# Srujan-D/spectral

Hardware: AMD Instinct MI355X
Metric: trajectory QP solves/sec (20-seg order-5 corridor) (higher is better)
Workload: dtype f64

## Files before the change

spectral_amd/csrc/btrapz_device.h:

```cpp
#ifndef BTRAPZ_DEVICE_H
#define BTRAPZ_DEVICE_H

#include "../../include/btrapz_hip.h"

#define BTRAPZ_EXPORT extern "C" __attribute__((visibility("default")))

#define BTRAPZ_FAR 1e9
#define BTRAPZ_FAR_FACTOR 1048576.0
#define BTRAPZ_FAR_LIMIT 1e6
#define BTRAPZ_COLD_FAR 1e4

namespace btrapz {

struct Shared {
  double w_s[4], w_l[4];
  double weight_end_s, weight_end_l;
  double ds_ref, dl_ref;
  double acc_s[2];
  double acc_l[2];
  double jerk_s[2], jerk_l[2];
  int variant;
};

struct KernelArgs {
// ... 124 lines not shown
  double rate;
  double s_lo, s_hi, l_lo, l_hi, l_safe, w_safe;
};

struct CorridorArgs {
  int B, N, num_obs, variant, seg_stride;
  double delta;
  const double *s_bounds, *l_bounds;
  const double *prisms;
  int P;
  PrismRoad road;
  int *n_strips;
  const double *ds_bounds, *dl_bounds;
  const double *s_ref, *l_ref;
  double *seg;
  int *seg_count;
  double *ref_end;
  double *dl10;
  int cap_o, cap_sel;
  int pass;
  int *retry_list, *retry_count;
};

__global__ void corridor_batch_kernel(const CorridorArgs a, int staged);
__global__ void corridor_batch_short_kernel(const CorridorArgs a, int staged);
__global__ void corridor_first_kernel(const CorridorArgs a, int staged);
__global__ void corridor_first_short_kernel(const CorridorArgs a, int staged);
__global__ void prism_corridor_batch_kernel(const CorridorArgs a, int staged);
__global__ void prism_corridor_batch_short_kernel(const CorridorArgs a, int staged);
__global__ void prism_corridor_first_kernel(const CorridorArgs a, int staged);
__global__ void prism_corridor_first_short_kernel(const CorridorArgs a, int staged);
struct Seg;
__global__ void corridor_serial_kernel(const CorridorArgs a, Seg *ws_all, Seg *ws_sel);
struct CorridorVjpArgs {
  int B, N, num_obs, variant, seg_stride;
  double delta;
  const double *s_bounds, *l_bounds, *ds_bounds, *s_ref, *l_ref;
  const double *seg_bar, *ref_end_bar, *dl10_bar;
  btrapz_knot_grads out;
  int cap_o, cap_sel, pass, staged;
  int *retry_list, *retry_count;
};
constexpr int kCorridorVjpTerms = 16;
struct CorridorVjpLds { int rows; size_t sel, dyn, ints, bytes; };
__host__ __device__ inline CorridorVjpLds corridor_vjp_lds(int N, int O, int cap_o, int cap_sel, int seg_stride, int staged) {
  CorridorVjpLds l;
  const size_t cap_all = (size_t)cap_o * O, seg_bytes = 104;
  l.rows = (cap_sel < seg_stride ? cap_sel : seg_stride) + 1;
  const size_t terms = (size_t)kCorridorVjpTerms * l.rows * (sizeof(double) + sizeof(int));
  l.sel = ((seg_bytes * cap_all > terms ? seg_bytes * cap_all : terms) + 15) & ~(size_t)15;
  l.dyn = (l.sel + seg_bytes * cap_sel + 15) & ~(size_t)15;
  const size_t table = staged ? (size_t)O * N * 2 : 0, refs = (size_t)N * 4;
  l.ints = l.dyn + sizeof(double) * (table > refs ? table : refs);
  l.bytes = l.ints + sizeof(int) * (64 + 4) + sizeof(short) * (cap_all + cap_sel);
  return l;
}
__global__ void corridor_vjp_kernel(const CorridorVjpArgs a);
__global__ void prestart_kernel(const KernelArgs a, int S_uniform, const int *seg_count, int *keys);
__global__ void bucket_hist_kernel(int B, int seg_stride, const int *seg_count, int *meta, int fixed_S);
__global__ void bucket_prefix_kernel(int *meta, int fixed_S);
__global__ void bucket_scatter_kernel(int B, int seg_stride, const int *seg_count, int *meta, int *order,
                                      double *axis_obj, int *axis_status, int *axis_iters, int fixed_S);
__global__ void ipm_solve_kernel(const KernelArgs a, const double *__restrict__ mqm);
__global__ void ipm_solve_ordered_kernel(const KernelArgs a, const double *__restrict__ mqm);
__global__ void ipm_solve_warm_kernel(const KernelArgs a, const double *__restrict__ mqm);
__global__ void ipm_solve_warm_ordered_kernel(const KernelArgs a, const double *__restrict__ mqm);
#ifdef BTRAPZ_EXPERIMENTS
__global__ void ipm_solve_queue_kernel(const KernelArgs a, const double *__restrict__ mqm);
#endif
__global__ void ipm_solve_elastic_kernel(const KernelArgs a, const double *__restrict__ mqm);
__global__ void ipm_solve_split_kernel(const KernelArgs a, const double *__restrict__ mqm);
__global__ void ipm_solve_capped_kernel(const KernelArgs a, const double *__restrict__ mqm);
__global__ void ipm_solve_capped_ordered_kernel(const KernelArgs a, const double *__restrict__ mqm);
__global__ void ipm_solve_resume_kernel(const KernelArgs a, const double *__restrict__ mqm);
__global__ void ipm_solve_lean_kernel(const KernelArgs a, const double *__restrict__ mqm);
__global__ void ipm_solve_lean_ordered_kernel(const KernelArgs a, const double *__restrict__ mqm);
__global__ void ipm_solve_lean_capped_kernel(const KernelArgs a, const double *__restrict__ mqm);
__global__ void ipm_solve_lean_capped_ordered_kernel(const KernelArgs a, const double *__restrict__ mqm);
__global__ void ipm_solve_lean_resume_kernel(const KernelArgs a, const double *__restrict__ mqm);
__global__ void ipm_solve_lean_pipe_capped_kernel(const KernelArgs a, const double *__restrict__ mqm, int axis);
__global__ void ipm_solve_lean_pipe_resume_kernel(const KernelArgs a, const double *__restrict__ mqm, int axis);
__global__ void ipm_solve_lean_pipe_kernel(const KernelArgs a, const double *__restrict__ mqm, int n_resume, int resume_axis, int capped_axis);
__global__ void pipe_counts_kernel(const int *tables, volatile int *host_counts);
__global__ void ipm_solve_lean_warm_kernel(const KernelArgs a, const double *__restrict__ mqm);
__global__ void ipm_solve_lean_warm_ordered_kernel(const KernelArgs a, const double *__restrict__ mqm);
__global__ void ipm_solve_sets_ordered_kernel(const KernelArgs a, const double *__restrict__ mqm, const Shared *sets, int n_keys);
__global__ void ipm_solve_sets_warm_ordered_kernel(const KernelArgs a, const double *__restrict__ mqm, const Shared *sets, int n_keys);
__global__ void ipm_solve_lean_sets_ordered_kernel(const KernelArgs a, const double *__restrict__ mqm, const Shared *sets, int n_keys);
__global__ void ipm_solve_lean_sets_warm_ordered_kernel(const KernelArgs a, const double *__restrict__ mqm, const Shared *sets, int n_keys);
__global__ void ipm_solve_sets_split_kernel(const KernelArgs a, const double *__restrict__ mqm, const Shared *sets, const int *set_index, int n_sets);
__global__ void ipm_solve_long_sets_kernel(const KernelArgs a, const double *__restrict__ mqm, const Shared *sets, const int *set_index, int n_sets);
__global__ void sets_hist_kernel(int B, int seg_stride, const int *seg_count, const int *set_index, int n_sets, int n_keys, int *meta);
__global__ void sets_prefix_kernel(int n_keys, int fixed_S, int *meta);
__global__ void sets_scatter_kernel(int B, int seg_stride, const int *seg_count, const int *set_index, int n_sets, int n_keys,
                                    int *meta, int *order, double *axis_obj, int *axis_status, int *axis_iters);
#define BTRAPZ_SUSPENDED (-7)
__global__ void ipm_solve_long_kernel(const KernelArgs a, const double *__restrict__ mqm);
__global__ void ipm_solve_long_elastic_kernel(const KernelArgs a, const double *__restrict__ mqm);
__global__ void rescue_keys_kernel(int B, int S, const int *seg_count, const int *axis_status, int *keys, int all);
__global__ void rescue_init_kernel(int B, int S, const int *seg_count, double *axis_obj, int *axis_status, int *axis_iters);
struct MqmWeights { double w[2][4]; };
__global__ void mqm_table_kernel(MqmWeights w, double *out);
__global__ void mqm_sets_kernel(const Shared *sets, double *out);
__global__ void rescue_violations_kernel(int B, const double *axis_viol, double *viol);
__global__ void finalize_kernel(int B, const double *axis_obj, const int *axis_status, const int *axis_iters,
                                double *cost, int *status, int *iters);
__global__ void argmin_kernel(int group, long long index_base, const double *cost, long long *best_idx,
                              double *best_cost, double *part_cost, long long *part_idx);
__global__ void argmin_final_kernel(int chunks, long long index_base, const double *part_cost, const long long *part_idx,
                                    long long *best_idx, double *best_cost);
__global__ void argmin_pairs_kernel(int world, int n, const long long *pairs, double *best_cost, long long *best_idx);
__global__ void eval_states_kernel(int B, int seg_stride, const int *seg_count, const double *seg, const double *ctrl,
                                   int n_times, const double *times, double *x);
__global__ void sample_kernel(int B, int seg_stride, const int *seg_count, double delta, const double *seg,
                              const double *init, const double *ctrl, int nsel, const long long *sel, int max_points,
                              double *out, int *npoints);

__global__ void single_candidate_kernel(const KernelArgs a, const double *__restrict__ mqm, double delta, int max_points,
                                        double *out);
__global__ void single_candidate_split_kernel(const KernelArgs a, const double *__restrict__ mqm, double delta, int max_points,
                                              double *out);
__global__ void single_candidate_warm_split_kernel(const KernelArgs a, const double *__restrict__ mqm, double delta, int max_points,
                                                   double *out);
__global__ void single_candidate_warm_kernel(const KernelArgs a, const double *__restrict__ mqm, double delta, int max_points,
                                             double *out);

}

int btrapz_ctx_device(const btrapz_ctx *ctx);
void btrapz_ctx_set_error(btrapz_ctx *ctx, const char *what);
int btrapz_launch_single(btrapz_ctx *ctx, const btrapz_shared *shared, const btrapz_options *opt, int S, const double *in,
                         double *out, int max_points, int warm, void *stream);
void btrapz_single_forget(btrapz_ctx *ctx);
void btrapz_mqm_table_host(const btrapz_shared *shared, double *table );
#endif
```

spectral_amd/csrc/btrapz_host.hip:

```cpp
#include <hip/hip_runtime.h>

#include <cmath>
#include <cstdio>
#include <cstdlib>
#include <cstring>
#include <string>
#include <vector>

#include <cstddef>
#include <type_traits>
#include "btrapz_device.h"
#include "btrapz_select.h"
#include "corridor_jvp.h"
#include "../../include/btrapz_hip_stage_jvp.h"
#include "../../include/btrapz_hip_schedule.h"
#include "prism_core.h"

using namespace btrapz;

static inline const char *experiment_env(const char *name) {
#ifdef BTRAPZ_EXPERIMENTS
  return getenv(name);
#else
  (void)name;
  return nullptr;
#endif
}

#define BTRAPZ_DEFAULT_STEP_FRACTION 0.9999
#define BTRAPZ_DEFAULT_STEP_THRESHOLD 0.9
#define BTRAPZ_AGGRESSIVE_ITERATIONS 12
#define BTRAPZ_STALL_START 10
#define BTRAPZ_STALL_LENGTH 6
#define BTRAPZ_STALL_FACTOR 0.8f
#define BTRAPZ_DIVERGE_FACTOR 1e3f
#define BTRAPZ_DEFAULT_ELASTIC_DELTA 1e-8
#define BTRAPZ_DEFAULT_ELASTIC_TOL 0.0125
#ifndef BTRAPZ_CAP_ALONE
#define BTRAPZ_CAP_ALONE 1
#endif
#ifndef BTRAPZ_CAP_HI
#define BTRAPZ_CAP_HI 4
#endif
#ifndef BTRAPZ_CAP_SCORE
#define BTRAPZ_CAP_SCORE 0.0
#endif
#ifndef BTRAPZ_SUSP_PERCENT
#define BTRAPZ_SUSP_PERCENT 15
#endif
#define BTRAPZ_SUSP_BYTES_MAX (1ull << 30)
#ifndef BTRAPZ_PIPELINE
#define BTRAPZ_PIPELINE 1
#endif
#define BTRAPZ_PIPELINE_RATIO 4

static_assert(offsetof(btrapz::Shared, acc_l) == offsetof(btrapz::Shared, acc_s) + 2 * sizeof(double) &&
              offsetof(btrapz::Shared, jerk_s) == offsetof(btrapz::Shared, acc_s) + 4 * sizeof(double) &&
              offsetof(btrapz::Shared, jerk_l) == offsetof(btrapz::Shared, acc_s) + 6 * sizeof(double), "Shared: acc_s, acc_l, jerk_s, jerk_l contiguous");
static_assert(std::is_trivially_copyable<btrapz::KernelArgs>::value && alignof(btrapz::KernelArgs) <= 8, "KernelArgs is passed by value at kernarg offset 0");

struct DevBuf {
  void *p = nullptr;
  size_t bytes = 0;
  explicit DevBuf(std::vector<DevBuf *> &owner) { owner.push_back(this); }
  DevBuf(const DevBuf &) = delete;
  void release() { (void)hipFree(p); p = nullptr; bytes = 0; }
  __attribute__((always_inline)) hipError_t grow(size_t need) { return need <= bytes ? hipSuccess : regrow(need); }
  __attribute__((noinline)) hipError_t regrow(size_t need) {
    release();
    const hipError_t e = hipMalloc(&p, need);
    if (e == hipSuccess) bytes = need; else p = nullptr;
    return e;
  }
};
template <class T> struct Buf : DevBuf {
  using DevBuf::DevBuf;
  T *ptr() const { return static_cast<T *>(p); }
  operator T *() const { return ptr(); }
  size_t cap() const { return bytes / sizeof(T); }
};
template <class... B> static void release_all(B &...b) { (b.release(), ...); }

struct btrapz_ctx {
  int device = 0;
  std::string err;
  std::vector<DevBuf *> bufs;
  Buf<double> d_axis_obj{bufs};
  Buf<double> d_axis_viol{bufs};
  Buf<int> d_axis_status{bufs}, d_axis_iters{bufs};
  size_t viol_valid = 0;
  Buf<double> d_mqm{bufs};
  double h_mqm_w[8] = {NAN, NAN, NAN, NAN, NAN, NAN, NAN, NAN};
  Buf<int> d_order{bufs};
  Buf<int> d_meta{bufs};
  Buf<int> d_retry{bufs};
  Buf<char> d_strips{bufs};
  Buf<char> d_corr_ws{bufs};
  Buf<int> d_vjp_retry{bufs};
  Buf<int> d_long_list{bufs};
  hipEvent_t ws_free = nullptr; hipStream_t ws_stream = nullptr; bool ws_used = false;
  Buf<double> d_argmin_cost{bufs}; Buf<long long> d_argmin_idx{bufs};
  Buf<double> d_topk_cost{bufs}; Buf<long long> d_topk_idx{bufs};
  Buf<int> d_rescue{bufs};
  Buf<int> d_rescue_meta{bufs};
  Buf<double> d_stage{bufs};
  Buf<int> d_istage{bufs};
  Buf<double> d_single{bufs};
  Buf<double> d_single_warm{bufs}; int single_S = 0, single_variant = -1, single_flip = 0;
  Buf<int> d_queue{bufs};
  Buf<double> d_susp_state{bufs};
  Buf<int> d_susp_ints{bufs};
  int resident_waves = 1024;
  int last_form = -1;
  int last_launches = 0;
  int *h_pipe_counts = nullptr; hipEvent_t pipe_landed = nullptr; bool pipe_pending = false;
  int pipe_pending_S = 0, pipe_pending_variant = -1;
  int pipe_S = 0, pipe_variant = -1, pipe_count[2] = {0, 0};
  int schedule_mode = 0;
  Buf<Shared> d_sets{bufs}; Buf<double> d_mqm_sets{bufs}; size_t sets_cap = 0;
  std::vector<Shared> h_sets;
  Shared *h_sets_stage[2] = {nullptr, nullptr}; hipEvent_t sets_copied[2] = {nullptr, nullptr};
  bool sets_copy_pending[2] = {false, false}; int sets_stage_next = 0;
  Buf<int> d_sets_meta{bufs};
  Buf<double> d_mqm_unit{bufs};
};

#define HIPCHK_AS(ctx, what, call)                                                            \
  do {                                                                                        \
    hipError_t e_ = (call);                                                                   \
    if (e_ != hipSuccess) {                                                                   \
      (ctx)->err = std::string(what) + ": " + hipGetErrorString(e_);                          \
      return BTRAPZ_EHIP;                                                                     \
    }                                                                                         \
  } while (0)
#define HIPCHK(ctx, call) HIPCHK_AS(ctx, #call, call)
#define GROW(ctx, buf, nbytes) HIPCHK_AS(ctx, "hipMalloc(&c->" #buf ", " #nbytes ")", (ctx)->buf.grow(nbytes))
#define TRY(call) do { const int rc_ = (call); if (rc_ != BTRAPZ_OK) return rc_; } while (0)
// ... 121 lines not shown
  a.tau = (opt && opt->step_fraction > 0 && opt->step_fraction < 1) ? opt->step_fraction : BTRAPZ_DEFAULT_STEP_FRACTION;
  a.tau_iters = BTRAPZ_AGGRESSIVE_ITERATIONS;
  a.stall_start = BTRAPZ_STALL_START; a.stall_len = BTRAPZ_STALL_LENGTH;
  static const float stall_factor_env = [] { const char *v = experiment_env("BTRAPZ_STALL_FACTOR"); return v ? (float)atof(v) : 0.0f; }();
  a.stall_factor = stall_factor_env > 0.0f ? stall_factor_env : BTRAPZ_STALL_FACTOR;
  a.diverge_factor = BTRAPZ_DIVERGE_FACTOR;
  a.tau_thr = (opt && opt->step_threshold > 0) ? opt->step_threshold : BTRAPZ_DEFAULT_STEP_THRESHOLD;
  a.x0 = warm ? warm->x0 : nullptr; a.lam0 = warm ? warm->lam0 : nullptr; a.lam_out = warm ? warm->lam_out : nullptr;
  a.mu0 = (warm && warm->mu0 > 0) ? warm->mu0 : 1e-4;
  a.smin = (warm && warm->smin > 0) ? warm->smin : 1e-2;
  a.elastic_delta = (opt && opt->elastic_delta > 0) ? opt->elastic_delta : BTRAPZ_DEFAULT_ELASTIC_DELTA;
  a.elastic_tol = (opt && opt->elastic_tol > 0) ? opt->elastic_tol : BTRAPZ_DEFAULT_ELASTIC_TOL;
  a.bucket_S = 0;
  a.cap_iter = 0; a.cap_alone = 0; a.cap_hi = 0; a.cap_score = 0.0; a.susp_cap = 0; a.susp_state = nullptr; a.susp_count = nullptr; a.susp_slot = nullptr; a.susp_key = nullptr;
#ifdef BTRAPZ_EXPERIMENTS
  static const int start_env = [] { const char *e = experiment_env("BTRAPZ_START"); return e ? atoi(e) : -1; }();
  a.unc_start = start_env >= 0 ? start_env : (opt ? opt->start : 0);
#else
  a.unc_start = 0;
#endif
}

void btrapz_mqm_table_host(const btrapz_shared *sh, double *table) {
#pragma clang fp contract(off)
  static const double M[6][6] = {{1, 0, 0, 0, 0, 0},      {-5, 5, 0, 0, 0, 0},      {10, -20, 10, 0, 0, 0},
                                 {-10, 30, -30, 10, 0, 0}, {5, -20, 30, -20, 5, 0}, {-1, 5, -10, 10, -5, 1}};
  for (int axis = 0; axis < 2; axis++) {
    const double *w = axis == 0 ? sh->w_s : sh->w_l;
    for (int d = 0; d < 4; d++)
      for (int j = 0; j < 6; j++)
        for (int i = 0; i <= j; i++) {
          double acc = 0.0;
          for (int a = d; a < 6; a++) {
            double t = 0.0;
            for (int b = d; b < 6; b++) {
              double num = w[d];
              for (int r = 0; r < d; r++) num *= double((a - r) * (b - r));
              t += num / double(a + b - 2 * d + 1) * M[b][j];
            }
            acc += M[a][i] * t;
          }
          table[(axis * 4 + d) * 21 + j * (j + 1) / 2 + i] = acc;
        }
  }
}

static void launch_mqm_table(hipStream_t stream, const double *w_s, const double *w_l, double *table) {
  MqmWeights mw;
  memcpy(mw.w[0], w_s, sizeof(double) * 4); memcpy(mw.w[1], w_l, sizeof(double) * 4);
  hipLaunchKernelGGL(mqm_table_kernel, dim3(1), dim3(192), 0, stream, mw, table);
}

void btrapz_single_forget(btrapz_ctx *c) { if (c) c->single_S = 0; }

BTRAPZ_EXPORT int btrapz_debug_mqm_tables(btrapz_ctx *c, const btrapz_shared *sh, double *host_table, double *device_table) {
  if (!c || !sh || !host_table || !device_table) return BTRAPZ_EINVAL;
  HIPCHK(c, hipSetDevice(c->device));
  btrapz_mqm_table_host(sh, host_table);
  double *d = nullptr;
  HIPCHK(c, hipMalloc(&d, sizeof(double) * 168));
  launch_mqm_table(nullptr, sh->w_s, sh->w_l, d);
  hipError_t e = hipMemcpy(device_table, d, sizeof(double) * 168, hipMemcpyDeviceToHost);
  (void)hipFree(d);
  HIPCHK(c, e);
  return BTRAPZ_OK;
}

BTRAPZ_EXPORT int btrapz_debug_axis_records(btrapz_ctx *c, int B, int *iters, int *status) {
  if (!c || B < 1 || (size_t)2 * B > c->d_axis_iters.cap() || !iters || !status) return BTRAPZ_EINVAL;
  HIPCHK(c, hipSetDevice(c->device));
  HIPCHK(c, hipDeviceSynchronize());
  HIPCHK(c, hipMemcpy(iters, c->d_axis_iters, sizeof(int) * 2 * B, hipMemcpyDeviceToHost));
  HIPCHK(c, hipMemcpy(status, c->d_axis_status, sizeof(int) * 2 * B, hipMemcpyDeviceToHost));
  return BTRAPZ_OK;
}
BTRAPZ_EXPORT int btrapz_debug_resume_keys(btrapz_ctx *c, int B, int *keys) {
  if (!c || B < 1 || !keys || c->d_susp_ints.cap() < 400 + 4 * (size_t)B) return BTRAPZ_EINVAL;
  HIPCHK(c, hipSetDevice(c->device));
  HIPCHK(c, hipDeviceSynchronize());
  HIPCHK(c, hipMemcpy(keys, c->d_susp_ints + 400, sizeof(int) * 2 * B, hipMemcpyDeviceToHost));
  return BTRAPZ_OK;
}
BTRAPZ_EXPORT int btrapz_debug_set_schedule(btrapz_ctx *c, int mode) {
  if (!c || mode < -1 || mode > 2) return BTRAPZ_EINVAL;
  c->schedule_mode = mode;
  return BTRAPZ_OK;
}
BTRAPZ_EXPORT int btrapz_debug_solve_launches(const btrapz_ctx *c) { return c ? c->last_launches : -1; }

int btrapz_launch_single(btrapz_ctx *c, const btrapz_shared *sh, const btrapz_options *opt, int S, const double *in,
                         double *out, int max_points, int warm, void *stream_) {
  hipStream_t stream = (hipStream_t)stream_;
  if (!c || !sh || S < 1 || S > BTRAPZ_MAX_SEGMENTS || !in || !out || max_points < 1 || !options_ok(c, opt)) return BTRAPZ_EINVAL;
  HIPCHK(c, hipSetDevice(c->device));
  KernelArgs a;
  fill_parameters(a, sh, opt, nullptr);
  a.B = 1; a.S = S; a.seg_stride = S; a.order = nullptr; a.seg_count = nullptr; a.cand_prefix = nullptr; a.wave_prefix = nullptr;
  const double *mqm = in + (size_t)BTRAPZ_NUM_SEG_FIELDS * S + 18;
  a.seg = in; a.init = in + (size_t)BTRAPZ_NUM_SEG_FIELDS * S; a.ref_end = a.init + 6; a.dl_bounds = a.ref_end + 2; a.mqm = mqm;
  TRY(ensure_axis_ws(c, 2));
  GROW(c, d_single, sizeof(double) * 12 * BTRAPZ_MAX_SEGMENTS);
  TRY(ws_wait(c, stream));
  a.axis_obj = c->d_axis_obj; a.axis_status = c->d_axis_status; a.axis_iters = c->d_axis_iters;
  a.ctrl = c->d_single; a.queue = nullptr; a.x_out = nullptr; a.axis_viol = nullptr;
  const bool split_form = S <= 21 && !(opt && opt->split < 0);
  if (warm) {
    const size_t nx = 2 * 64 * 3, nl = 2 * 36 * 64, set = nx + nl;
    GROW(c, d_single_warm, sizeof(double) * 2 * set);
    double *rd = c->d_single_warm + (size_t)c->single_flip * set, *wr = c->d_single_warm + (size_t)(1 - c->single_flip) * set;
    const bool have = c->single_S == S && c->single_variant == sh->variant;
    a.x0 = have ? rd : nullptr; a.lam0 = have ? rd + nx : nullptr;
    a.x_out = wr; a.lam_out = wr + nx;
    c->single_flip = 1 - c->single_flip; c->single_S = S; c->single_variant = sh->variant;
  }
  auto kernel = warm ? (split_form ? single_candidate_warm_split_kernel : single_candidate_warm_kernel)
                     : (split_form ? single_candidate_split_kernel : single_candidate_kernel);
  hipLaunchKernelGGL(kernel, dim3(1), dim3(128), 0, stream, a, mqm, sh->delta, max_points, out);
  TRY(ws_close(c, stream));
  HIPCHK(c, hipGetLastError());
  return BTRAPZ_OK;
}


static void launch_bucket_lists(hipStream_t stream, unsigned ny, int B, int S, const int *keys, int *tables, int *lists,
                                double *obj, int *status, int *iters, int fixed_S) {
  const unsigned nb = (unsigned)((B + 255) / 256);
  hipLaunchKernelGGL(bucket_hist_kernel, dim3(nb, ny), dim3(256), 0, stream, B, S, keys, tables, fixed_S);
  hipLaunchKernelGGL(bucket_prefix_kernel, dim3(1, ny), dim3(64), 0, stream, tables, fixed_S);
  hipLaunchKernelGGL(bucket_scatter_kernel, dim3(nb, ny), dim3(256), 0, stream, B, S, keys, tables, lists, obj, status, iters, fixed_S);
}

struct FormQuery {
  int B, S, elastic, max_iter, unc_start, resident_waves;
  bool ragged, warm_kernel, ordered, compact;
  int split, lean, cap_iter; bool queue;
  unsigned blocks;
};
struct Form { bool long_form, split_on, lean_on, capped, queue_on; int cap_iter; };

static Form choose_form(const FormQuery &q) {
  Form f;
  f.long_form = !q.ragged && q.S > BTRAPZ_MAX_SEGMENTS;
  f.queue_on = q.queue;
  f.split_on = !q.ordered && !q.warm_kernel && q.S <= 21 &&
               (q.split > 0 || (q.split == 0 && 2u * (unsigned)q.B <= (unsigned)q.resident_waves));
  const bool lean_ok = !f.long_form && !f.split_on && !f.queue_on && (q.S >= 3 || q.ragged) && q.S <= BTRAPZ_MAX_SEGMENTS && q.unc_start == 0;
  const unsigned est_waves = 2u * (unsigned)((size_t)q.B / (size_t)(64 / (q.S < 64 ? q.S : 64)) + 1);
  f.lean_on = lean_ok && (q.lean > 0 || (q.lean == 0 && 4u * est_waves >= 5u * (unsigned)q.resident_waves));
  f.cap_iter = q.cap_iter;
  if (f.cap_iter == 0 && !q.ragged && q.S >= 16 && q.S <= 32 && q.blocks >= 8u * (unsigned)q.resident_waves) f.cap_iter = 6;
  f.capped = f.cap_iter > 0 && !f.long_form && !f.split_on && (!q.ordered || q.ragged || q.compact) && !q.warm_kernel && !f.queue_on && q.S <= BTRAPZ_MAX_SEGMENTS &&
             f.cap_iter < q.max_iter && f.cap_iter + BTRAPZ_CAP_HI < 4000 && q.elastic != 2;
  return f;
}

template <class Launch>
static int solve_long_candidates(btrapz_ctx *c, hipStream_t stream, const KernelArgs &a, const int *seg_count, Launch launch) {
  const int B = a.B, S = a.S;
  std::vector<int> counts((size_t)B);
  HIPCHK(c, hipMemcpyAsync(counts.data(), seg_count, sizeof(int) * (size_t)B, hipMemcpyDeviceToHost, stream));
  HIPCHK(c, hipStreamSynchronize(stream));
  const int smax = S < BTRAPZ_MAX_SEGMENTS_LONG ? S : BTRAPZ_MAX_SEGMENTS_LONG;
  std::vector<std::vector<int>> by_count((size_t)smax + 1);
  size_t n_long = 0;
  for (int b = 0; b < B; b++)
    if (counts[b] > BTRAPZ_MAX_SEGMENTS && counts[b] <= smax) { by_count[(size_t)counts[b]].push_back(b); ++n_long; }
  if (!n_long) return BTRAPZ_OK;
// ... 69 lines not shown
    HIPCHK(c, hipGetLastError());
  }
  if (seg_count || hint || s.compact) {
    GROW(c, d_order, sizeof(int) * (size_t)B);
    GROW(c, d_meta, sizeof(int) * 198);
    HIPCHK(c, hipMemsetAsync(c->d_meta, 0, sizeof(int) * 198, s.stream));
    const int fixed_S = seg_count ? 0 : (s.compact ? -S : S);
    const int *keys = s.compact ? compact_keys : seg_count ? seg_count : hint;
    launch_bucket_lists(s.stream, 1, B, S, keys, c->d_meta, c->d_order, s.compact ? (double *)nullptr : c->d_axis_obj.ptr(),
                        s.compact ? (int *)nullptr : c->d_axis_status.ptr(), s.compact ? (int *)nullptr : c->d_axis_iters.ptr(), fixed_S);
    HIPCHK(c, hipGetLastError());
    a.order = c->d_order; a.seg_count = seg_count; a.cand_prefix = c->d_meta; a.wave_prefix = c->d_meta + 66;
    a.bucket_S = seg_count ? 0 : S;
    const int gpw_min = seg_count ? 1 : 64 / S;
    s.blocks = 2u * (unsigned)(B / gpw_min + 65);
  } else {
    const int gpw = S <= 64 ? 64 / S : 1;
    s.blocks = 2u * (unsigned)((B + gpw - 1) / gpw);
  }
  s.warm_kernel = a.x0 || a.lam0 || a.lam_out;
  return BTRAPZ_OK;
}

static void solve_requests(const btrapz_options *opt, FormQuery &q) {
#ifdef BTRAPZ_EXPERIMENTS
  static const int queue_env = [] { const char *q = experiment_env("BTRAPZ_QUEUE"); return q ? (*q == '0' ? -1 : 1) : 0; }();
  q.queue = queue_env ? queue_env > 0 : (opt && opt->queue > 0);
#else
  q.queue = false;
#endif
  const char *split_q = experiment_env("BTRAPZ_SPLIT");
  const int split_env = split_q ? (*split_q == '0' ? -1 : 1) : 0;
  q.split = split_env ? split_env : (opt ? opt->split : 0);
  static const int cap_env = [] { const char *q = experiment_env("BTRAPZ_CAP"); return q ? atoi(q) : -1; }();
  q.cap_iter = cap_env > 0 ? cap_env : cap_env == 0 ? -1 : (opt ? opt->cap_iter : 0);
  static const int lean_env = [] { const char *q = experiment_env("BTRAPZ_LEAN"); return q ? (*q == '0' ? -1 : 1) : 0; }();
  q.lean = lean_env ? lean_env : (opt ? opt->lean : 0);
}

static int capped_workspace(Solve &s, bool requested, size_t *slots_out) {
  btrapz_ctx *c = s.c; const size_t B = (size_t)s.B, S = (size_t)s.S;
  size_t slots = 2 * B * (size_t)BTRAPZ_SUSP_PERCENT / 100;
  if (slots < 1024) slots = 1024;
  const size_t slots_max = (size_t)BTRAPZ_SUSP_BYTES_MAX / (sizeof(double) * 74 * S);
  if (slots > slots_max) slots = slots_max;
  if (slots > (size_t)0x7fffffff) slots = (size_t)0x7fffffff;
  bool ok = slots >= 64;
  ok = ok && c->d_susp_state.grow(sizeof(double) * slots * 74 * S) == hipSuccess;
  ok = ok && c->d_susp_ints.grow(sizeof(int) * (400 + 4 * B)) == hipSuccess;
  ok = ok && c->d_rescue.grow(sizeof(int) * 4 * B) == hipSuccess;
  ok = ok && c->d_rescue_meta.grow(sizeof(int) * 2 * 198) == hipSuccess;
  if (!ok) {
    (void)hipGetLastError();
    if (requested) { c->err = "btrapz_options.cap_iter: no memory for the hand-over workspace"; return BTRAPZ_ENOMEM; }
  }
  *slots_out = ok ? slots : 0;
  return BTRAPZ_OK;
}

static int launch_capped_and_resume(Solve &s, const Form &f, size_t slots) {
  btrapz_ctx *c = s.c; const int B = s.B, S = s.S;
  const bool ragged = s.seg_count != nullptr;
  int *count = c->d_susp_ints, *tables = count + 4, *keys = tables + 2 * 198, *slot_of = keys + 2 * (size_t)B;
  HIPCHK(c, hipMemsetAsync(count, 0, sizeof(int) * (400 + 2 * (size_t)B), s.stream));
  KernelArgs p1 = s.a;
  p1.cap_iter = f.cap_iter; p1.cap_alone = BTRAPZ_CAP_ALONE; p1.cap_hi = f.cap_iter + BTRAPZ_CAP_HI; p1.cap_score = BTRAPZ_CAP_SCORE; p1.susp_cap = (int)slots; p1.susp_state = c->d_susp_state; p1.susp_count = count;
  p1.susp_slot = slot_of; p1.susp_key = keys;
  auto first = f.lean_on ? (p1.order ? ipm_solve_lean_capped_ordered_kernel : ipm_solve_lean_capped_kernel)
                         : (p1.order ? ipm_solve_capped_ordered_kernel : ipm_solve_capped_kernel);
  hipLaunchKernelGGL(first, dim3(s.blocks), dim3(64), 0, s.stream, p1, (const double *)c->d_mqm);
  int *lists = c->d_rescue + 2 * (size_t)B;
  const int list_S = ragged ? 0 : -S;
  launch_bucket_lists(s.stream, 2, B, S, keys, tables, lists, nullptr, nullptr, nullptr, list_S);
  KernelArgs p2 = p1;
  p2.cap_iter = 0; p2.order = lists; p2.seg_count = nullptr; p2.cand_prefix = tables; p2.wave_prefix = tables + 66;
  p2.bucket_S = ragged ? 0 : S;
  const unsigned rblocks = 2u * (unsigned)(slots / (size_t)(64 / (S < 64 ? S : 64)) + 65);
  hipLaunchKernelGGL(f.lean_on ? ipm_solve_lean_resume_kernel : ipm_solve_resume_kernel, dim3(rblocks), dim3(64), 0, s.stream, p2, (const double *)c->d_mqm);
  c->last_form = f.lean_on ? 11 : 3;
  c->last_launches = 2;
  return BTRAPZ_OK;
}

static int pipeline_first_axis(btrapz_ctx *c, int S, int variant) {
#if BTRAPZ_PIPELINE
  if (c->schedule_mode != 0) return c->schedule_mode < 0 ? -1 : c->schedule_mode - 1;
  if (c->pipe_pending) {
    if (hipEventQuery(c->pipe_landed) == hipSuccess) {
      c->pipe_pending = false;
      c->pipe_S = c->pipe_pending_S; c->pipe_variant = c->pipe_pending_variant;
      c->pipe_count[0] = c->h_pipe_counts[0]; c->pipe_count[1] = c->h_pipe_counts[1];
    } else {
      (void)hipGetLastError();
    }
  }
  if (c->pipe_S != S || c->pipe_variant != variant) return -1;
  const long long n0 = c->pipe_count[0], n1 = c->pipe_count[1];
  if (n0 > 0 && n0 >= BTRAPZ_PIPELINE_RATIO * n1) return 0;
  if (n1 > 0 && n1 >= BTRAPZ_PIPELINE_RATIO * n0) return 1;
#endif
  return -1;
}

static void pipeline_remember(Solve &s, const int *tables, int variant) {
#if BTRAPZ_PIPELINE
  btrapz_ctx *c = s.c;
  if (!c->h_pipe_counts) {
    if (hipHostMalloc((void **)&c->h_pipe_counts, sizeof(int) * 2, hipHostMallocDefault) != hipSuccess) { c->h_pipe_counts = nullptr; (void)hipGetLastError(); return; }
    c->h_pipe_counts[0] = 0; c->h_pipe_counts[1] = 0;
  }
  if (!c->pipe_landed && hipEventCreateWithFlags(&c->pipe_landed, hipEventDisableTiming) != hipSuccess) { c->pipe_landed = nullptr; (void)hipGetLastError(); return; }
  hipLaunchKernelGGL(pipe_counts_kernel, dim3(1), dim3(64), 0, s.stream, tables, c->h_pipe_counts);
  if (hipEventRecord(c->pipe_landed, s.stream) != hipSuccess) { (void)hipGetLastError(); c->pipe_pending = false; c->pipe_S = 0; return; }
  c->pipe_pending = true; c->pipe_pending_S = s.S; c->pipe_pending_variant = variant;
#else
  (void)s; (void)tables; (void)variant;
#endif
}

static int launch_pipelined(Solve &s, const Form &f, size_t slots, int a0) {
  btrapz_ctx *c = s.c; const int B = s.B, S = s.S, a1 = 1 - a0;
  int *count = c->d_susp_ints, *tables = count + 4, *keys = tables + 2 * 198, *slot_of = keys + 2 * (size_t)B;
  HIPCHK(c, hipMemsetAsync(count, 0, sizeof(int) * (400 + 2 * (size_t)B), s.stream));
  int *lists = c->d_rescue + 2 * (size_t)B;
  KernelArgs p = s.a;
  p.cap_iter = f.cap_iter; p.cap_alone = BTRAPZ_CAP_ALONE; p.cap_hi = f.cap_iter + BTRAPZ_CAP_HI; p.cap_score = BTRAPZ_CAP_SCORE; p.susp_cap = (int)slots; p.susp_state = c->d_susp_state; p.susp_count = count;
  p.susp_slot = slot_of; p.susp_key = keys;
  p.order = lists; p.seg_count = nullptr; p.cand_prefix = tables; p.wave_prefix = tables + 66; p.bucket_S = S;
  const int gpw = 64 / S;
  const unsigned cblocks = (unsigned)((B + gpw - 1) / gpw);
  const unsigned rblocks = (unsigned)(slots / (size_t)gpw + 65);
  auto bucket = [&](int ax) {
    launch_bucket_lists(s.stream, 1, B, S, keys + (size_t)ax * B, tables + ax * 198, lists + (size_t)ax * B, nullptr, nullptr, nullptr, -S);
  };
  hipLaunchKernelGGL(ipm_solve_lean_pipe_capped_kernel, dim3(cblocks), dim3(64), 0, s.stream, p, (const double *)c->d_mqm, a0);
  bucket(a0);
  hipLaunchKernelGGL(ipm_solve_lean_pipe_kernel, dim3(rblocks + cblocks), dim3(64), 0, s.stream, p, (const double *)c->d_mqm, (int)rblocks, a0, a1);
  bucket(a1);
  hipLaunchKernelGGL(ipm_solve_lean_pipe_resume_kernel, dim3(rblocks), dim3(64), 0, s.stream, p, (const double *)c->d_mqm, a1);
  c->last_form = 11;
  c->last_launches = 3;
  return BTRAPZ_OK;
}

static int solve_main_launch(Solve &s, Form &f) {
  btrapz_ctx *c = s.c; KernelArgs &a = s.a;
  const int B = s.B, S = s.S;
  c->last_launches = 1;
  FormQuery q{};
  q.B = B; q.S = S; q.ragged = s.seg_count != nullptr; q.warm_kernel = s.warm_kernel; q.ordered = a.order != nullptr; q.compact = s.compact;
  q.elastic = s.elastic; q.max_iter = a.max_iter; q.unc_start = a.unc_start; q.resident_waves = c->resident_waves; q.blocks = s.blocks;
  solve_requests(s.opt, q);
  f = choose_form(q);
  if (f.long_form && (a.order || s.warm_kernel || s.elastic == 2 || (s.elastic == 1 && S > BTRAPZ_MAX_SEGMENTS_LONG_RESCUE))) {
    c->err = "more than 64 segments: uniform cold solve only, rescue pass (elastic = 1) up to 192 segments";
    return BTRAPZ_EINVAL;
  }
  if (s.elastic == 2) return BTRAPZ_OK;
  size_t slots = 0;
  if (f.capped) TRY(capped_workspace(s, q.cap_iter > 0, &slots));
  if (slots) {
    const bool pipe_ok = f.lean_on && !s.seg_count && !a.order;
    const int first_axis = pipe_ok ? pipeline_first_axis(c, S, a.sh.variant) : -1;
    if (first_axis >= 0) TRY(launch_pipelined(s, f, slots, first_axis));
    else TRY(launch_capped_and_resume(s, f, slots));
    if (pipe_ok) pipeline_remember(s, c->d_susp_ints + 4, a.sh.variant);
  } else if (f.long_form) {
    c->last_form = 2;
    hipLaunchKernelGGL(ipm_solve_long_kernel, dim3(2u * (unsigned)B), dim3(64u * (unsigned)((S + 63) / 64)), 0, s.stream, a, (const double *)c->d_mqm);
  } else if (f.split_on) {
    c->last_form = 1;
    hipLaunchKernelGGL(ipm_solve_split_kernel, dim3(2u * (unsigned)B), dim3(64), 0, s.stream, a, (const double *)c->d_mqm);
#ifdef BTRAPZ_EXPERIMENTS
  } else if (f.queue_on && !a.order && !s.warm_kernel && s.blocks >= 3u * (unsigned)c->resident_waves) {
    HIPCHK(c, hipMemsetAsync(c->d_queue, 0, sizeof(int) * 2, s.stream));
    c->last_form = 4;
    hipLaunchKernelGGL(ipm_solve_queue_kernel, dim3((unsigned)c->resident_waves & ~1u), dim3(64), 0, s.stream, a, (const double *)c->d_mqm);
#endif
  } else if (f.lean_on) {
    c->last_form = 8;
    auto lean_kernel = s.warm_kernel ? (a.order ? ipm_solve_lean_warm_ordered_kernel : ipm_solve_lean_warm_kernel)
                                     : (a.order ? ipm_solve_lean_ordered_kernel : ipm_solve_lean_kernel);
    hipLaunchKernelGGL(lean_kernel, dim3(s.blocks), dim3(64), 0, s.stream, a, (const double *)c->d_mqm);
  } else {
    c->last_form = 0;
    auto kernel = s.warm_kernel ? (a.order ? ipm_solve_warm_ordered_kernel : ipm_solve_warm_kernel)
                                : (a.order ? ipm_solve_ordered_kernel : ipm_solve_kernel);
    hipLaunchKernelGGL(kernel, dim3(s.blocks), dim3(64), 0, s.stream, a, (const double *)c->d_mqm);
  }
  HIPCHK(c, hipGetLastError());
  return BTRAPZ_OK;
}

static KernelArgs rescue_arguments(const KernelArgs &a) {
  KernelArgs e = a;
  e.x0 = nullptr; e.lam0 = nullptr; e.lam_out = nullptr;
  e.max_iter = a.max_iter < 120 ? 120 : a.max_iter;
  e.tau_iters = 0;
  e.stall_start = 4 * BTRAPZ_STALL_START; e.stall_len = 4 * BTRAPZ_STALL_LENGTH;
  return e;
}

static int solve_rescue_pass(Solve &s, bool long_form) {
  btrapz_ctx *c = s.c; const int B = s.B, S = s.S;
  if (long_form) {
    HIPCHK(c, hipMemsetAsync(c->d_axis_viol, 0, sizeof(double) * 8 * (size_t)B, s.stream));
    c->viol_valid = (size_t)B;
    KernelArgs e = rescue_arguments(s.a);
    e.order = nullptr;
    hipLaunchKernelGGL(ipm_solve_long_elastic_kernel, dim3(2u * (unsigned)B), dim3(64u * (unsigned)((S + 63) / 64)), 0, s.stream, e, (const double *)c->d_mqm);
    HIPCHK(c, hipGetLastError());
    return BTRAPZ_OK;
  }
  GROW(c, d_rescue, sizeof(int) * 4 * (size_t)B);
  GROW(c, d_rescue_meta, sizeof(int) * 2 * 198);
  HIPCHK(c, hipMemsetAsync(c->d_axis_viol, 0, sizeof(double) * 8 * (size_t)B, s.stream));
  c->viol_valid = (size_t)B;
  int *keys = c->d_rescue, *lists = c->d_rescue + 2 * (size_t)B;
  const unsigned nb = (unsigned)((B + 255) / 256);
  if (s.elastic == 2)
    hipLaunchKernelGGL(rescue_init_kernel, dim3(nb), dim3(256), 0, s.stream, B, S, s.seg_count, c->d_axis_obj,
                       c->d_axis_status, c->d_axis_iters);
  hipLaunchKernelGGL(rescue_keys_kernel, dim3(nb), dim3(256), 0, s.stream, B, S, s.seg_count, (const int *)c->d_axis_status,
                     keys, s.elastic == 2 ? 1 : 0);
  HIPCHK(c, hipMemsetAsync(c->d_rescue_meta, 0, sizeof(int) * 2 * 198, s.stream));
  for (int ax = 0; ax < 2; ax++)
    launch_bucket_lists(s.stream, 1, B, S, keys + (size_t)ax * B, c->d_rescue_meta + ax * 198, lists + (size_t)ax * B, nullptr, nullptr, nullptr, 0);
  HIPCHK(c, hipGetLastError());
  KernelArgs e = rescue_arguments(s.a);
  e.order = lists; e.seg_count = s.seg_count; e.cand_prefix = c->d_rescue_meta; e.wave_prefix = c->d_rescue_meta + 66;
  e.bucket_S = 0;
  const int smax = s.seg_count ? (S < 64 ? S : 64) : S;
  const unsigned eblocks = 2u * (unsigned)(B / (64 / smax) + 65);
  hipLaunchKernelGGL(ipm_solve_elastic_kernel, dim3(eblocks), dim3(64), 0, s.stream, e, (const double *)c->d_mqm);
  HIPCHK(c, hipGetLastError());
  return BTRAPZ_OK;
}

static int solve_common(btrapz_ctx *c, const btrapz_shared *sh, const btrapz_options *opt, const btrapz_warm *warm,
                        int B, int S, const int *seg_count, const double *seg, const double *init, const double *ref_end,
                        const double *dl_bounds, double *ctrl, double *cost, int *status, int *iters, void *stream_) {
  if (!c) return BTRAPZ_EINVAL;
  if (!sh || B < 1 || S < 1 || (!seg_count && S > BTRAPZ_MAX_SEGMENTS_LONG) || !seg || !init || !ref_end || !dl_bounds ||
      !ctrl || !cost || !status) {
    c->err = "invalid argument";
    return BTRAPZ_EINVAL;
  }
  if (!options_ok(c, opt)) return BTRAPZ_EINVAL;
  Solve s;
// ... 807 lines not shown
```

spectral_amd/native.py:

```python
import ctypes as C
import os
import subprocess

import numpy as np

from . import layout as L

_HERE = os.path.dirname(os.path.abspath(__file__))
LIB_DIR = os.path.join(_HERE, "lib")
CSRC_DIR = os.path.join(_HERE, "csrc")
LIB_PATH = os.environ.get("BTRAPZ_HIP_LIB") or os.path.join(LIB_DIR, "libbtrapz_hip.so")


class BtrapzError(RuntimeError):
    pass


class CShared(C.Structure):
    _fields_ = [("w_s", C.c_double * 4), ("w_l", C.c_double * 4),
                ("weight_end_s", C.c_double), ("weight_end_l", C.c_double),
                ("ds_ref", C.c_double), ("dl_ref", C.c_double),
                ("dds", C.c_double * 2), ("ddds", C.c_double * 2),
                ("ddl", C.c_double * 2), ("dddl", C.c_double * 2),
                ("delta", C.c_double), ("variant", C.c_int), ("reserved", C.c_int)]
# ... 148 lines not shown
    "btrapz_solve_ragged_device": (_i, [_vp, _sh, _opt, _i, _i] + _ragged + _result + [_vp]),
    "btrapz_corridor_batch_device": (_i, [_vp, _i, _i, _i, _i, _d] + _knots + [_i, _vp, _vp, _vp, _vp, _vp]),
    "btrapz_corridor_batch_vjp_device": (_i, [_vp, _i, _i, _i, _i, _d] + _knots + [_i, _vp, _vp, _vp, C.POINTER(CKnotGrads), _vp]),
    "btrapz_corridor_vjp_host": (_i, [_i, _i, _i, _d] + _knots + [_i, _vp, _vp, _vp, C.POINTER(CKnotGrads), _ip]),
    "btrapz_prism_bounds_device": (_i, [_vp, _i, _i, _i, _road, _vp, _i, _vp, _vp, _vp, _vp]),
    "btrapz_prism_bounds_vjp_device": (_i, [_vp, _i, _i, _i, _road, _vp, _i, _vp, _vp, _vp, _vp]),
    "btrapz_prism_bounds_vjp_host": (_i, [_i, _i, _i, _road, _vp, _i, _vp, _vp, _vp]),
    "btrapz_prism_corridor_batch_device": (_i, [_vp, _i, _i, _i, _i, _road, _vp, _i, _d, _vp, _vp, _vp, _vp, _i, _vp, _vp, _vp,
                                                _vp, _vp, _vp]),
    "btrapz_solve_warm_device": (_i, [_vp, _sh, _opt, C.POINTER(CWarm), _i, _i] + _ragged + _result + [_vp]),
    "btrapz_solve_sets_device": (_i, [_vp, _sh, _i, _vp, _opt, C.POINTER(CWarm), _i, _i] + _ragged + _result + [_vp]),
    "btrapz_solve_vjp_device": (_i, [_vp, _sh, _i, _vp, _i, _i] + _ragged + [_vp, _vp, _vp, _vp, _vp, C.POINTER(CGrads), _vp]),
    "btrapz_solve_jvp_device": (_i, [_vp, _sh, _i, _vp, _i, _i] + _ragged + [_vp, _vp, _vp, _i, C.POINTER(CTangents), _vp, _vp,
                                     _vp]),
    "btrapz_traj_cost_device": (_i, [_vp, _sh, _i, _vp, _i, _i, _vp, _vp, _vp, _vp, _vp, _i, _vp, _vp, _i, _vp, _vp, _vp]),
    "btrapz_traj_cost_vjp_device": (_i, [_vp, _sh, _i, _vp, _i, _i, _vp, _vp, _vp, _vp, _vp, _i, _vp, _vp, _i] + [_vp] * 7),
    "btrapz_eval_states_device": (_i, [_vp, _i, _i, _vp, _vp, _vp, _i, _vp, _vp, _vp]),
    "btrapz_sample_vjp_device": (_i, [_vp, _i, _i, _vp, _d, _vp, _i, _vp, _i, _vp, _vp, _vp, _vp]),
    "btrapz_eval_states_vjp_device": (_i, [_vp, _i, _i, _vp, _vp, _vp, _i, _vp, _vp, _vp, _vp, _vp]),
    "btrapz_debug_mqm_tables": (_i, [_vp, _sh, _vp, _vp]),
    "btrapz_debug_axis_records": (_i, [_vp, _i, _vp, _vp]),
    "btrapz_debug_resume_keys": (_i, [_vp, _i, _vp]),
    "btrapz_debug_parse_double": (_d, [_str, _ip]),
    "btrapz_debug_format_fixed": (_i, [_d, _str]),
}
EXPORTS = tuple(PROTOTYPES)

PROTOTYPES_STAGE_JVP = {
    "btrapz_prism_bounds_jvp_device": (_i, [_vp, _i, _i, _i, _road, _vp, _i, _i, _vp, _vp, _vp, _vp]),
    "btrapz_prism_bounds_jvp_host": (_i, [_i, _i, _i, _road, _vp, _i, _i, _vp, _vp, _vp]),
    "btrapz_corridor_batch_jvp_device": (_i, [_vp, _i, _i, _i, _i, _d] + _knots + [_i, _i, C.POINTER(CKnotTangents), _vp, _vp, _vp, _vp]),
    "btrapz_corridor_jvp_host": (_i, [_i, _i, _i, _d] + _knots + [_i, _i, C.POINTER(CKnotTangents), _vp, _vp, _vp, _ip]),
}
EXPORTS_STAGE_JVP = tuple(PROTOTYPES_STAGE_JVP)

PROTOTYPES_SCHEDULE = {
    "btrapz_debug_set_schedule": (_i, [_vp, _i]),
    "btrapz_debug_solve_launches": (_i, [_vp]),
}
EXPORTS_SCHEDULE = tuple(PROTOTYPES_SCHEDULE)

PROTOTYPES_SELECT = {
    "btrapz_topk_device": (_i, [_vp, _i, _i, _i, _ll, _vp, _vp, _vp, _vp]),
    "btrapz_topk_pairs_device": (_i, [_vp, _i, _i, _i, _vp, _vp, _vp, _vp]),
    "btrapz_gather_rows_device": (_i, [_vp, _i, _vp, _ll, _i, _i, _vp, _vp, _vp]),
}
EXPORTS_SELECT = tuple(PROTOTYPES_SELECT)
MAX_TOPK = 64


def _ptr(t):
    return C.c_void_p(t.data_ptr()) if t is not None else None


def _np_ptr(a):
    return a.ctypes.data_as(C.c_void_p) if a is not None else None


def _np_f64(a):
    return None if a is None else np.ascontiguousarray(a, dtype=np.float64)


def _stream(stream):
    return C.c_void_p(stream or 0)


def _sets_array(sets):
    return (CShared * max(len(sets), 1))(*[CShared.from_shared(sh) for sh in sets])


def _warm(x0, lam0, lam_out, mu0, smin, hint):
    return CWarm(_ptr(x0), _ptr(lam0), _ptr(lam_out), float(mu0), float(smin), _ptr(hint))


def build(verbose=False):
    out = None if verbose else subprocess.DEVNULL
    subprocess.check_call(["make", "-j4", "-C", CSRC_DIR, "all"], stdout=out)
    return LIB_PATH


def kernel_source_hash():
    import hashlib
    h = hashlib.sha256()
    for f in ("btrapz_kernels.hip", "btrapz_lean.hip", "btrapz_lean_warm.hip", "btrapz_lean_pipe.hip", "btrapz_lean_body.h", "btrapz_ipm.h", "btrapz_device.h", "Makefile",
              os.path.join("..", "..", "include", "btrapz_hip.h")):
        with open(os.path.join(CSRC_DIR, f), "rb") as fh:
            h.update(fh.read())
    return h.hexdigest()[:16]


_lib = None
ROCM_HIP_RUNTIME = "/opt/rocm/lib/libamdhip64.so"


def _bind_hip_runtime():
    import sys
    path = ROCM_HIP_RUNTIME
    if "torch" in sys.modules:
        bundled = os.path.join(os.path.dirname(sys.modules["torch"].__file__), "lib", "libamdhip64.so")
        if os.path.exists(bundled):
            path = bundled
    try:
        C.CDLL(path, mode=C.RTLD_GLOBAL)
    except OSError as e:
        raise BtrapzError("cannot load the HIP runtime %s: %s (there is no CPU path)" % (path, e))


def lib():
    global _lib
    if _lib is None:
        if not os.path.exists(LIB_PATH):
            raise BtrapzError("HIP library %s is missing: run spectral_amd.native.build() "
                              "(there is no CPU path)" % LIB_PATH)
        _bind_hip_runtime()
        l = C.CDLL(LIB_PATH)
        for name, (restype, argtypes) in list(PROTOTYPES.items()) + list(PROTOTYPES_STAGE_JVP.items()) + list(PROTOTYPES_SCHEDULE.items()) + list(PROTOTYPES_SELECT.items()):
            fn = getattr(l, name)
            fn.restype, fn.argtypes = restype, argtypes
        _lib = l
    return _lib


def multi_shard_bounds(B, G, g, group=0):
    lo, hi = C.c_int(0), C.c_int(0)
    rc = lib().btrapz_multi_shard_bounds(int(B), int(G), int(g), int(group), C.byref(lo), C.byref(hi))
    if rc != 0:
        raise BtrapzError("btrapz_multi_shard_bounds(%d, %d, %d, %d) -> %d" % (B, G, g, group, rc))
    return lo.value, hi.value


class MultiContext:

    def __init__(self, devices, transport=MULTI_AUTO):
        self._h = C.c_void_p()
        devs = (C.c_int * len(devices))(*[int(d) for d in devices])
        rc = lib().btrapz_multi_create(C.byref(self._h), devs, len(devices), int(transport))
        if rc != 0:
            raise BtrapzError("btrapz_multi_create(%s, transport=%d) failed with %d (no HIP device, or the transport "
                              "cannot be had: see stderr)" % (list(devices), transport, rc))
        self.G = len(devices); self.B = self.S = 0; self.group = 0

    def close(self):
        if self._h:
            lib().btrapz_multi_destroy(self._h)
            self._h = C.c_void_p()

    def __del__(self):
        try:
            self.close()
        except Exception:
            pass

    def _check(self, rc, what):
        if rc != 0:
            raise BtrapzError("%s failed (%d): %s" % (what, rc, lib().btrapz_multi_last_error(self._h).decode()))

    def transport(self):
        return int(lib().btrapz_multi_transport(self._h))

    def transport_library(self):
        return lib().btrapz_multi_transport_library(self._h).decode()

    def fallback_reason(self):
        return lib().btrapz_multi_last_error(self._h).decode()

    def upload(self, batch, group=0):
        seg, init, ref_end, dlb = _np_f64(batch.seg), _np_f64(batch.init), _np_f64(batch.ref_end), _np_f64(batch.dl_bounds)
# ... 427 lines not shown
```

Before: 18.34 million.

## Add quiet-axis schedule running one axis uncapped alongside resumed capped axis

Adds a new schedule for the case where one axis almost never hits the iteration cap (count ratio of at least 256). That axis runs through a plain lean solve with no capping, fused into the same launch as the resume pass of the other, capped axis. This removes the capped and resume overhead on the quiet axis. A new counts kernel estimates how often the quiet axis would have needed capping, so the schedule can switch back. The Makefile is not shown, so whether the new source file is compiled is uncertain.

```diff
diff --git a/spectral_amd/csrc/btrapz_device.h b/spectral_amd/csrc/btrapz_device.h
--- a/spectral_amd/csrc/btrapz_device.h
+++ b/spectral_amd/csrc/btrapz_device.h
@@ -230,6 +230,10 @@
 __global__ void ipm_solve_lean_pipe_resume_kernel(const KernelArgs a, const double *__restrict__ mqm, int axis);
 __global__ void ipm_solve_lean_pipe_kernel(const KernelArgs a, const double *__restrict__ mqm, int n_resume, int resume_axis, int capped_axis);
 __global__ void pipe_counts_kernel(const int *tables, volatile int *host_counts);
+__global__ void ipm_solve_lean_quiet_plain_kernel(const KernelArgs a, const double *__restrict__ mqm, int axis);
+__global__ void ipm_solve_lean_quiet_kernel(const KernelArgs a, const double *__restrict__ mqm, int n_resume, int resume_axis, int plain_axis);
+__global__ void quiet_counts_kernel(const int *__restrict__ axis_iters, int B, int gpw, int quiet_axis, int cap_iter, int cap_hi,
+                                    const int *tables, int *acc, volatile int *host_counts);
 __global__ void ipm_solve_lean_warm_kernel(const KernelArgs a, const double *__restrict__ mqm);
 __global__ void ipm_solve_lean_warm_ordered_kernel(const KernelArgs a, const double *__restrict__ mqm);
 __global__ void ipm_solve_sets_ordered_kernel(const KernelArgs a, const double *__restrict__ mqm, const Shared *sets, int n_keys);
diff --git a/spectral_amd/csrc/btrapz_host.hip b/spectral_amd/csrc/btrapz_host.hip
--- a/spectral_amd/csrc/btrapz_host.hip
+++ b/spectral_amd/csrc/btrapz_host.hip
@@ -53,6 +53,7 @@
 #define BTRAPZ_PIPELINE 1
 #endif
 #define BTRAPZ_PIPELINE_RATIO 4
+#define BTRAPZ_QUIET_RATIO 256
 
 static_assert(offsetof(btrapz::Shared, acc_l) == offsetof(btrapz::Shared, acc_s) + 2 * sizeof(double) &&
               offsetof(btrapz::Shared, jerk_s) == offsetof(btrapz::Shared, acc_s) + 4 * sizeof(double) &&
@@ -340,7 +341,7 @@
   return BTRAPZ_OK;
 }
 BTRAPZ_EXPORT int btrapz_debug_set_schedule(btrapz_ctx *c, int mode) {
-  if (!c || mode < -1 || mode > 2) return BTRAPZ_EINVAL;
+  if (!c || mode < -1 || mode > 4) return BTRAPZ_EINVAL;
   c->schedule_mode = mode;
   return BTRAPZ_OK;
 }
@@ -576,7 +577,7 @@
   return BTRAPZ_OK;
 }
 
-static int pipeline_first_axis(btrapz_ctx *c, int S, int variant) {
+static int pipeline_schedule(btrapz_ctx *c, int S, int variant) {
 #if BTRAPZ_PIPELINE
   if (c->schedule_mode != 0) return c->schedule_mode < 0 ? -1 : c->schedule_mode - 1;
   if (c->pipe_pending) {
@@ -590,25 +591,35 @@
   }
   if (c->pipe_S != S || c->pipe_variant != variant) return -1;
   const long long n0 = c->pipe_count[0], n1 = c->pipe_count[1];
+  if (n0 > 0 && n0 >= BTRAPZ_QUIET_RATIO * n1) return 2;
+  if (n1 > 0 && n1 >= BTRAPZ_QUIET_RATIO * n0) return 3;
   if (n0 > 0 && n0 >= BTRAPZ_PIPELINE_RATIO * n1) return 0;
   if (n1 > 0 && n1 >= BTRAPZ_PIPELINE_RATIO * n0) return 1;
 #endif
   return -1;
 }
 
-static void pipeline_remember(Solve &s, const int *tables, int variant) {
+static void pipeline_remember(Solve &s, int *count, int variant, int quiet_axis, int cap_iter) {
 #if BTRAPZ_PIPELINE
   btrapz_ctx *c = s.c;
+  const int *tables = count + 4;
   if (!c->h_pipe_counts) {
     if (hipHostMalloc((void **)&c->h_pipe_counts, sizeof(int) * 2, hipHostMallocDefault) != hipSuccess) { c->h_pipe_counts = nullptr; (void)hipGetLastError(); return; }
     c->h_pipe_counts[0] = 0; c->h_pipe_counts[1] = 0;
   }
   if (!c->pipe_landed && hipEventCreateWithFlags(&c->pipe_landed, hipEventDisableTiming) != hipSuccess) { c->pipe_landed = nullptr; (void)hipGetLastError(); return; }
-  hipLaunchKernelGGL(pipe_counts_kernel, dim3(1), dim3(64), 0, s.stream, tables, c->h_pipe_counts);
+  if (quiet_axis < 0) {
+    hipLaunchKernelGGL(pipe_counts_kernel, dim3(1), dim3(64), 0, s.stream, tables, c->h_pipe_counts);
+  } else {
+    const int gpw = 64 / s.S;
+    const unsigned waves = (unsigned)((s.B + gpw - 1) / gpw);
+    hipLaunchKernelGGL(quiet_counts_kernel, dim3((waves + 255u) / 256u), dim3(256), 0, s.stream, (const int *)s.a.axis_iters, s.B, gpw, quiet_axis,
+                       cap_iter, cap_iter + BTRAPZ_CAP_HI, tables, count + 1, c->h_pipe_counts);
+  }
   if (hipEventRecord(c->pipe_landed, s.stream) != hipSuccess) { (void)hipGetLastError(); c->pipe_pending = false; c->pipe_S = 0; return; }
   c->pipe_pending = true; c->pipe_pending_S = s.S; c->pipe_pending_variant = variant;
 #else
-  (void)s; (void)tables; (void)variant;
+  (void)s; (void)count; (void)variant; (void)quiet_axis; (void)cap_iter;
 #endif
 }
 
@@ -637,6 +648,26 @@
   return BTRAPZ_OK;
 }
 
+static int launch_quiet_axis(Solve &s, const Form &f, size_t slots, int a0) {
+  btrapz_ctx *c = s.c; const int B = s.B, S = s.S, a1 = 1 - a0;
+  int *count = c->d_susp_ints, *tables = count + 4, *keys = tables + 2 * 198, *slot_of = keys + 2 * (size_t)B;
+  HIPCHK(c, hipMemsetAsync(count, 0, sizeof(int) * (400 + 2 * (size_t)B), s.stream));
+  int *lists = c->d_rescue + 2 * (size_t)B;
+  KernelArgs p = s.a;
+  p.cap_iter = f.cap_iter; p.cap_alone = BTRAPZ_CAP_ALONE; p.cap_hi = f.cap_iter + BTRAPZ_CAP_HI; p.cap_score = BTRAPZ_CAP_SCORE; p.susp_cap = (int)slots; p.susp_state = c->d_susp_state; p.susp_count = count;
+  p.susp_slot = slot_of; p.susp_key = keys;
+  p.order = lists; p.seg_count = nullptr; p.cand_prefix = tables; p.wave_prefix = tables + 66; p.bucket_S = S;
+  const int gpw = 64 / S;
+  const unsigned cblocks = (unsigned)((B + gpw - 1) / gpw);
+  const unsigned rblocks = (unsigned)(slots / (size_t)gpw + 65);
+  hipLaunchKernelGGL(ipm_solve_lean_pipe_capped_kernel, dim3(cblocks), dim3(64), 0, s.stream, p, (const double *)c->d_mqm, a0);
+  launch_bucket_lists(s.stream, 1, B, S, keys + (size_t)a0 * B, tables + a0 * 198, lists + (size_t)a0 * B, nullptr, nullptr, nullptr, -S);
+  hipLaunchKernelGGL(ipm_solve_lean_quiet_kernel, dim3(rblocks + cblocks), dim3(64), 0, s.stream, p, (const double *)c->d_mqm, (int)rblocks, a0, a1);
+  c->last_form = 11;
+  c->last_launches = 3;
+  return BTRAPZ_OK;
+}
+
 static int solve_main_launch(Solve &s, Form &f) {
   btrapz_ctx *c = s.c; KernelArgs &a = s.a;
   const int B = s.B, S = s.S;
@@ -655,10 +686,11 @@
   if (f.capped) TRY(capped_workspace(s, q.cap_iter > 0, &slots));
   if (slots) {
     const bool pipe_ok = f.lean_on && !s.seg_count && !a.order;
-    const int first_axis = pipe_ok ? pipeline_first_axis(c, S, a.sh.variant) : -1;
-    if (first_axis >= 0) TRY(launch_pipelined(s, f, slots, first_axis));
+    const int schedule = pipe_ok ? pipeline_schedule(c, S, a.sh.variant) : -1;
+    if (schedule >= 2) TRY(launch_quiet_axis(s, f, slots, schedule - 2));
+    else if (schedule >= 0) TRY(launch_pipelined(s, f, slots, schedule));
     else TRY(launch_capped_and_resume(s, f, slots));
-    if (pipe_ok) pipeline_remember(s, c->d_susp_ints + 4, a.sh.variant);
+    if (pipe_ok) pipeline_remember(s, c->d_susp_ints, a.sh.variant, schedule >= 2 ? 3 - schedule : -1, f.cap_iter);
   } else if (f.long_form) {
     c->last_form = 2;
     hipLaunchKernelGGL(ipm_solve_long_kernel, dim3(2u * (unsigned)B), dim3(64u * (unsigned)((S + 63) / 64)), 0, s.stream, a, (const double *)c->d_mqm);
diff --git a/spectral_amd/csrc/btrapz_lean_quiet.hip b/spectral_amd/csrc/btrapz_lean_quiet.hip
--- /dev/null
+++ b/spectral_amd/csrc/btrapz_lean_quiet.hip
@@ -0,0 +1,60 @@
+#include "btrapz_lean_body.h"
+
+namespace btrapz {
+
+LEAN_KERNEL void ipm_solve_lean_quiet_plain_kernel(const KernelArgs a, const double *__restrict__ mqm, int axis) {
+  __shared__ double lds[LN_ROWS][64];
+  lean_solve_body<false, false, false>(a, mqm, lds, 2 * (int)blockIdx.x + axis, (int)threadIdx.x);
+}
+
+LEAN_KERNEL void ipm_solve_lean_quiet_kernel(const KernelArgs, const double *__restrict__ mqm, int n_resume, int resume_axis,
+                                             int plain_axis) {
+  __shared__ double lds[LN_ROWS][64];
+  typedef const KernelArgs __attribute__((address_space(4))) kargs_t;
+  kargs_t *kp = (kargs_t *)__builtin_amdgcn_kernarg_segment_ptr();
+  const int blk = (int)blockIdx.x;
+  KernelArgs a;
+  if (blk < n_resume) {
+    asm volatile("; resume part" : "+s"(kp));
+    __builtin_memcpy(&a, kp, sizeof(KernelArgs));
+    lean_solve_body<true, false, true>(a, mqm, lds, 2 * blk + resume_axis, (int)threadIdx.x);
+  } else {
+    asm volatile("; plain part" : "+s"(kp));
+    __builtin_memcpy(&a, kp, sizeof(KernelArgs));
+    lean_solve_body<false, false, false>(a, mqm, lds, 2 * (blk - n_resume) + plain_axis, (int)threadIdx.x);
+  }
+}
+
+__global__ __launch_bounds__(256) void quiet_counts_kernel(const int *__restrict__ axis_iters, int B, int gpw, int quiet_axis,
+                                                           int cap_iter, int cap_hi, const int *tables, int *acc,
+                                                           volatile int *host_counts) {
+  const long long w = (long long)blockIdx.x * blockDim.x + threadIdx.x;
+  const long long c0 = w * gpw;
+  int n_over = 0;
+  if (c0 < B) {
+    const int ng = (int)(B - c0 < gpw ? B - c0 : gpw);
+    int top = 0, second = 0, n_top = 0;
+    for (int g = 0; g < ng; g++) {
+      const int n = axis_iters[2 * (c0 + g) + quiet_axis];
+      if (n > top) { second = top; top = n; n_top = 1; }
+      else if (n == top) n_top++;
+      else if (n > second) second = n;
+      n_over += n >= cap_hi;
+    }
+    if (n_top == 1 && top < cap_hi && top > (second > 0 ? (second > cap_iter ? second : cap_iter) : 1)) n_over++;
+  }
+  for (int d = 32; d > 0; d >>= 1) n_over += __shfl_xor(n_over, d);
+  if ((threadIdx.x & 63) == 0) {
+    if (n_over) atomicAdd(&acc[0], n_over);
+    __threadfence();
+  }
+  __syncthreads();
+  if (threadIdx.x == 0) {
+    if (atomicAdd(&acc[1], 1) == (int)gridDim.x - 1) {
+      host_counts[quiet_axis] = atomicAdd(&acc[0], 0);
+      host_counts[1 - quiet_axis] = tables[(1 - quiet_axis) * 198 + 65];
+    }
+  }
+}
+
+}
diff --git a/spectral_amd/native.py b/spectral_amd/native.py
--- a/spectral_amd/native.py
+++ b/spectral_amd/native.py
@@ -254,7 +254,7 @@
 def kernel_source_hash():
     import hashlib
     h = hashlib.sha256()
-    for f in ("btrapz_kernels.hip", "btrapz_lean.hip", "btrapz_lean_warm.hip", "btrapz_lean_pipe.hip", "btrapz_lean_body.h", "btrapz_ipm.h", "btrapz_device.h", "Makefile",
+    for f in ("btrapz_kernels.hip", "btrapz_lean.hip", "btrapz_lean_warm.hip", "btrapz_lean_pipe.hip", "btrapz_lean_quiet.hip", "btrapz_lean_body.h", "btrapz_ipm.h", "btrapz_device.h", "Makefile",
               os.path.join("..", "..", "include", "btrapz_hip.h")):
         with open(os.path.join(CSRC_DIR, f), "rb") as fh:
             h.update(fh.read())
```

New measurement: 18.89 million, median of 6. 1.03x the previous value.
